# shijun18/H-DenseFormer

Hardware: AMD Instinct MI355X
Metric: train samples/sec on 4x128^3 volumes (higher is better)
Workload: dtype bf16

## Files before the change

h-denseformer_amd/csrc/api_ops.hip:

```cpp
#include <atomic>
#include <algorithm>
#include <cstdarg>
#include <cstring>

#include "../../include/hdf.h"
#include "conv_igemm.h"
#include "loss.h"
#include "optim.h"
#include "transformer.h"
#include "unet_ops.h"

static thread_local char g_err[1024] = "";
static std::atomic<int> g_cu_budget{256};
static int device_cus() {
  static std::atomic<int> cache[16];
  int dev = 0;
  if (hipGetDevice(&dev) != hipSuccess || dev < 0 || dev >= 16) return 256;
  int v = cache[dev].load(std::memory_order_relaxed);
  if (v > 0) return v;
  int n = 0;
  if (hipDeviceGetAttribute(&n, hipDeviceAttributeMultiprocessorCount, dev) != hipSuccess || n <= 0) return 256;
  if (n >= 8) n &= ~7;
  cache[dev].store(n, std::memory_order_relaxed);
  return n;
// ... 386 lines not shown
                          const float* mean, const float* rstd, float* partials, int N, int C, int Do, int Ho, int Wo,
                          hdf_stream stream) {
  HDF_CHECK_ARG(dout && idx && din && y && scale && shift && mean && rstd && partials, "maxpool_bwd_in: null argument");
  return hdf_launch_maxpool_bwd_in(dtype, dout, dout_pitch, idx, din, din_pitch, y, y_pitch, scale, shift, mean, rstd,
                                   partials, N, C, Do, Ho, Wo, (hipStream_t)stream);
}
int hdf_op_upsample_fwd(int dtype, const void* y, int64_t y_pitch, const float* scale, const float* shift, void* out,
                        int64_t out_pitch, int N, int C, int Di, int Hi, int Wi, hdf_stream stream) {
  return hdf_launch_upsample_fwd(dtype, y, y_pitch, scale, shift, out, out_pitch, N, C, Di, Hi, Wi,
                                 (hipStream_t)stream);
}
int hdf_op_upsample_bwd(int dtype, const void* dout, int64_t dout_pitch, void* din, int64_t din_pitch, int N, int C,
                        int Di, int Hi, int Wi, hdf_stream stream) {
  return hdf_launch_upsample_bwd(dtype, dout, dout_pitch, din, din_pitch, N, C, Di, Hi, Wi, (hipStream_t)stream);
}


namespace {
TfDims op_dims(int M, int B, int N, int DM, int64_t mstride, int training, uint64_t seed) {
  TfDims d;
  d.M = M, d.B = B, d.N = N, d.DM = DM, d.DMF = DM + 128;
  d.mstride = mstride;
  d.training = training ? 1 : 0;
  d.seed = (uint32_t)(seed & 0xffffffffu);
  d.thresh24 = 1u << 23;
  d.keep_scale = 2.0f;
  return d;
}
int op_dims_ok(int M, int B, int N, int DM) {
  HDF_CHECK_ARG(M >= 1 && B >= 1 && N >= 1, "transformer op: M=%d B=%d N=%d", M, B, N);
// ... 106 lines not shown
```

h-denseformer_amd/csrc/exec.hip:

```cpp
#include <algorithm>
#include <cstring>
#include <map>
#include <string>

#include "plan_internal.h"
#include "loss.h"
#include "transformer.h"
#include "unet_ops.h"

namespace {

hipStream_t make_stream(bool highest) {
  hipStream_t s = nullptr;
  int least = 0, greatest = 0;
  if (hipDeviceGetStreamPriorityRange(&least, &greatest) != hipSuccess ||
      hipStreamCreateWithPriority(&s, hipStreamNonBlocking, highest ? greatest : least) != hipSuccess) {
    if (hipStreamCreateWithFlags(&s, hipStreamNonBlocking) != hipSuccess) s = nullptr;
  }
  return s;
}

struct Exec {
  hdf_plan* p;
  char* ws;
// ... 692 lines not shown
  void* outs[4] = {out0, out1, out2, out3};
  Xf none;

  static const bool no_branch = getenv("HDF_NO_BRANCH_OVERLAP") != nullptr;
  Exec eb = e;
  hipStream_t bst = no_branch ? nullptr : e.fork_branch();
  if (bst) eb.st = bst, eb.on_branch = true;
  Rejoin rejoin{e, eb, bst != nullptr};
  const bool fused_at3 = !p->flat;
  const int flat = p->flat ? 1 : 0;
  const bool first_direct = bst && p->enc[0][0].Cin <= 4 &&
                            hdf_conv_first_takes(p->dtype, p->enc[0][0].Cin, p->enc[0][0].Cout, p->dims[0][0], p->dims[0][1],
                                                 p->dims[0][2], p->xin.pitch);
  hipStream_t pst = first_direct ? bst : e.st;
  if (first_direct) {
    HDF_TRY(hdf_launch_nchw_to_ndhwc(p->dtype, x, e.at(p->xin), batch, p->M, 16, p->vox(0), e.st));
    HDF_TRY(conv_forward(e, p->enc[0][0], p->xin, none));
  }
  HDF_TRY(hdf_launch_pack_batch(p->dtype, params, e.ws, p->pack_jobs.data(), (int)p->pack_jobs.size(), pst));
  if (p->tf_fwd_chain)
    HDF_TRY(tf_chain_pack(tf_dims(p, batch), tf_chain_params(p), p->nb, params, e.ws + p->tf_wpack, pst));
  hipEvent_t packed = bst ? e.order(pst, e.st, "the caller's stream behind the weight packs", first_direct) : nullptr;
  if (bst && !packed) return HDF_ERR_HIP;
  if (!first_direct) {
    HDF_TRY(hdf_launch_nchw_to_ndhwc(p->dtype, x, e.at(p->xin), batch, p->M, 16, p->vox(0), e.st));
    HDF_TRY(conv_forward(e, p->enc[0][0], p->xin, none));
  }
  const bool chain_first = first_direct && p->tf_fwd_chain;
  eb.tf_packed = first_direct ? nullptr : packed;
  if (chain_first) {
    HDF_TRY(transformer_forward(eb, x));
    if (!e.order(bst, e.st, "the caller's stream behind the branch stream's transformer (tf_done)")) return HDF_ERR_HIP;
  }
  e.conv_budget = (hdf_cu_budget() * 3 / 4) & ~7;
  HDF_TRY(conv_forward(e, p->enc[0][1], p->enc[0][0].y, xf_of(e, p->enc[0][0])));
  e.conv_budget = 0;
  if (!chain_first) HDF_TRY(transformer_forward(eb, x));
  if (packed) HDF_TRY(e.wait(bst, packed, "the branch stream behind the weight packs"));
  HDF_TRY(conv_forward(eb, p->deep, p->attnall, none));
  HDF_TRY(hdf_launch_upsample_fwd(p->dtype, eb.at(p->deep.y), p->deep.y.pitch, eb.f(p->deep.st.scale),
// ... 74 lines not shown
}

static int backward3d(hdf_plan* p, const float* x, const float* params, void* workspace, int64_t workspace_bytes,
                      const void* dout0, const void* dout1, const void* dout2, const void* dout3, float* grads,
                      int batch, int stages, hdf_stream stream, hipEvent_t* bev = nullptr) {
  HDF_CHECK_ARG(p->batch == batch, "backward: batch %d differs from the forward's %d", batch, p->batch);
  HDF_TRY(chain_flag_check(p));
  auto record = [&](int k, hipStream_t s) -> int {
    if (bev && hipEventRecord(bev[k], s) != hipSuccess) {
      hdf_set_error("backward: could not record the event of gradient bucket %d", k);
      return HDF_ERR_HIP;
    }
    return HDF_OK;
  };
  enum { BK_DEC = 0, BK_CHAIN = 1, BK_TF = 2, BK_ENC = 3, BK_ENC0 = 4 };
  auto record_joined = [&](int k, Exec& ex) -> int {
    if (!bev) return HDF_OK;
    if (ex.async && p->side) {
      if (!ex.order(ex.st, p->side, "the side stream behind the issuing stream (gradient bucket event)")) return HDF_ERR_HIP;
      return record(k, p->side);
    }
    return record(k, ex.st);
  };
  HDF_CHECK_ARG((size_t)workspace_bytes >= p->ws_bytes,
                "backward: workspace of %lld bytes holds a forward only (hdf_plan_workspace_bytes = %zu)",
                (long long)workspace_bytes, p->ws_bytes);
  Exec e{p, (char*)workspace, params, grads, batch, (hipStream_t)stream};
  static const bool no_async = getenv("HDF_NO_ASYNC_WGRAD") != nullptr;
  if (!no_async) {
    if (!p->side) p->side = make_stream(false);
// ... 76 lines not shown
      HDF_TRY(hdf_launch_wgrad_first(p->dtype, e.at(p->gA[k]), p->gA[k].pitch, c1.Cout, e.at(p->xin), p->xin.pitch, c1.Cin,
                                     e.B, p->dims[0][0], p->dims[0][1], p->dims[0][2], e.G(c1.w), 0, e.ws + p->wgrad_ws,
                                     p->wgrad_ws_bytes, e.wgrad_stream(), &fi));
      HDF_TRY(e.wgrad_done(p->gA[k]));
      first_fused = true;
    }
    if (!first_fused) {
      if (k > 0)
        HDF_TRY(norm_conv_backward(e, c1, p->gA[k], p->gY2[k], bsr, p->pooled[k - 1], none, &p->dP[k - 1], 0));
      else
        HDF_TRY(norm_conv_backward(e, c1, p->gA[k], p->gY2[k], bsr, p->xin, none, nullptr, 0));
    }
    if (k == 1) HDF_TRY(record_joined(BK_ENC, e));
    if (k == 0 && forked) {
      HDF_TRY(transformer_backward(eb, x));
      if (bev) {
        eb.join();
        HDF_TRY(record(BK_TF, eb.st));
      }
    }
  }

  if (!(stages & 6) || bev) e.join();
  HDF_TRY(record(BK_ENC0, e.st));
  }
  if (forked) {
    HDF_TRY(e.join_branch(eb));
    forked = false;
  } else {
    if (stages & 2) {
      HDF_TRY(upconv_chain_backward(e, batch));
      if (!(stages & 4) || bev) e.join();
      HDF_TRY(record(BK_CHAIN, e.st));
    }
    if (stages & 4) {
      HDF_TRY(transformer_backward(e, x));
      if (bev) {
        e.join();
        HDF_TRY(record(BK_TF, e.st));
      }
    }
  }
  e.join();
  if ((stages & 4) && p->tf_bwd_chain) {
    const unsigned* tmo = reinterpret_cast<const unsigned*>(e.ws + p->tf_sync) + (1 << 17) + p->M * batch * 32;
    hipLaunchKernelGGL(chain_poison_grads_kernel, dim3(1), dim3(256), 0, e.st, tmo, grads,
                       (int)std::min<int64_t>(p->total_floats, 4096));
    HDF_LAUNCH_CHECK();
  }
  return HDF_OK;
}

static int backward_any(hdf_plan* p, const float* x, const float* params, void* workspace, int64_t workspace_bytes,
                        const void* dout0, const void* dout1, const void* dout2, const void* dout3, float* grads,
                        int batch, int stages, hdf_stream stream, hipEvent_t* bev) {
  HDF_CHECK_ARG(p && x && params && workspace && grads, "backward: null argument");
  if (!p->is2d)
    return backward3d(p, x, params, workspace, workspace_bytes, dout0, dout1, dout2, dout3, grads, batch, stages, stream,
                      bev);
  HDF_CHECK_ARG(p->batch == batch && (size_t)workspace_bytes >= p->ws_bytes, "backward: batch / workspace mismatch");
  char* ws = (char*)workspace;
  hipStream_t st = (hipStream_t)stream;
  void* d3[4];
  const void* d2[4] = {dout0, dout1, dout2, dout3};
// ... 141 lines not shown
```

h-denseformer_amd/csrc/plan.hip:

```cpp
#include <cstdarg>
#include <cstring>

#include "plan_internal.h"
#include "transformer.h"

namespace {

void add_param(hdf_plan* p, const std::string& name, std::vector<int64_t> shape) {
  ParamInfo pi;
  pi.name = name;
  pi.shape = shape;
  pi.numel = 1;
  for (auto s : shape) pi.numel *= s;
  pi.offset = p->total_floats;
  p->total_floats += (pi.numel + 15) / 16 * 16;
  p->pidx[name] = (int64_t)p->params.size();
  p->params.push_back(pi);
}

void build_params(hdf_plan* p) {
  const int nf = p->nf, DM = p->DM;
  char buf[256];
  for (int m = 0; m < p->M; m++) {
    int64_t start = p->total_floats;
// ... 151 lines not shown
      Embed2dJob& last = p->ejobs.back();
      if (last.kind == 0 && last.stage == stage && last.off3 + last.n3 == pi.offset && last.off2 + last.n3 == q.offset) {
        last.n3 += n3;
        p->params2d.push_back(q);
        continue;
      }
    }
    p->ejobs.push_back(Embed2dJob{pi.offset, q.offset, n3, inner, (short)rep, (char)kind, stage});
    p->params2d.push_back(q);
  }
  HDF_CHECK_ARG((int)p->ejobs.size() <= HDF_MAX_EMBED_JOBS, "2-D plan: %d embedding jobs (max %d)", (int)p->ejobs.size(),
                HDF_MAX_EMBED_JOBS);
  return HDF_OK;
}

View mkview(hdf_plan* p, Bump& bp, const std::string& name, int lvl, int C, int batch) {
  View v;
  v.C = C;
  v.pitch = C;
  v.lvl = lvl;
  v.off = bp.take((size_t)batch * p->vox(lvl) * C * p->esz);
  if (!name.empty()) p->bufs[name] = v;
  return v;
}

}

View hdf_plan_subview(hdf_plan* p, const View& v, int c0, int C, const std::string& name) {
  View s = v;
  s.off = v.off + (size_t)c0 * p->esz;
// ... 7 lines not shown
  p->batch = B;
  p->bufs.clear();
  Bump bp;
  const int nf = p->nf;
  const int ch[4] = {nf, 2 * nf, 4 * nf, 8 * nf};
  auto conv_bufs = [&](Conv3& c) {
    c.y = mkview(p, bp, "y." + c.name, c.lvl, c.Cout, B);
    size_t s = (size_t)B * c.Cout * sizeof(float);
    c.st.mean = bp.take(s);
    c.st.rstd = bp.take(s);
    c.st.scale = bp.take(s);
    c.st.shift = bp.take(s);
    c.wf = bp.take((size_t)27 * round_up(c.Cout, 32) * c.CinP * p->esz);
    c.wd = bp.take((size_t)27 * round_up(c.CinP, 32) * round_up(c.Cout, 16) * p->esz);
  };
  p->xin = mkview(p, bp, "xin", 0, 16, B);
  const int64_t rows = (int64_t)p->M * B * p->Ntok;
  p->tf_F = bp.take((size_t)p->nb * rows * p->DMF * sizeof(float));
  p->tf_save = bp.take((size_t)p->nb * 4 * rows * 232 * sizeof(float));
  {
    TfDims dd{};
    dd.M = p->M;
    p->tf_wpack = bp.take(tf_chain_wpack_bytes(dd, p->nb));
    dd.B = B, dd.N = p->Ntok;
    p->tf_frag = bp.take(p->dtype == HDF_F32 ? 256 : tf_chain_frag_bytes(dd, p->nb));
  }
  p->tf_sync = bp.take((size_t)3 << 20);
  p->attnall = mkview(p, bp, "attnall", 4, p->M * p->DM, B);
  conv_bufs(p->deep);
  p->attnout = mkview(p, bp, "attnout", 3, 8 * nf, B);
  for (int k = 0; k < 3; k++) conv_bufs(p->up[k]);
// ... 126 lines not shown
  p->D = D, p->H = H, p->W = W;
  p->td = transformer_depth;
  p->nb = transformer_depth / 4;
  p->dtype = dtype;
  p->esz = hdf_esz(dtype);
  for (int l = 0; l < 5; l++) p->dims[l][0] = D >> l, p->dims[l][1] = H >> l, p->dims[l][2] = W >> l;
  p->flat = is2d && flat;
  if (p->flat)
    for (int l = 0; l < 5; l++) p->dims[l][0] = 1;
  p->DM = 4 * n_filters;
  p->DMF = p->DM + 128;
  p->Ntok = (D / 16) * (H / 16) * (W / 16);
  build_params(p);
  build_layers(p);
  p->is2d = is2d;
  if (is2d) {
    int rc = build_params2d(p);
    if (rc != HDF_OK) {
      delete p;
      return rc;
    }
  }
  *out = p;
  return HDF_OK;
}

int hdf_plan_create(int in_channels, int n_cls, int n_filters, int D, int H, int W, int transformer_depth, int dtype,
                    hdf_plan** out) {
  return create_plan(in_channels, n_cls, n_filters, D, H, W, transformer_depth, dtype, false, out);
}
// ... 36 lines not shown
  return (int64_t)p->ws_fwd_bytes;
}

int hdf_plan_buffer_info(hdf_plan* p, int batch, const char* name, int64_t* byte_offset, int64_t* pitch_elems,
                         int* channels, int* d, int* h, int* w) {
  hdf_plan_layout(p, batch);
  auto it = p->bufs.find(name);
  HDF_CHECK_ARG(it != p->bufs.end(), "buffer_info: no buffer named '%s'", name);
  const View& v = it->second;
  *byte_offset = (int64_t)v.off;
  *pitch_elems = v.pitch;
  *channels = v.C;
  *d = p->dims[v.lvl][0];
  *h = p->dims[v.lvl][1];
  *w = p->dims[v.lvl][2];
  return HDF_OK;
}

int hdf_plan_region_info(hdf_plan* p, int batch, const char* name, int64_t* byte_offset, int64_t* bytes) {
  HDF_CHECK_ARG(p && name && byte_offset && bytes, "region_info: null argument");
  hdf_plan_layout(p, batch);
  const int64_t rows = (int64_t)p->M * batch * p->Ntok;
  const std::string n = name;
  if (n == "tf_F") *byte_offset = (int64_t)p->tf_F, *bytes = (int64_t)p->nb * rows * p->DMF * 4;
  else if (n == "tf_save") *byte_offset = (int64_t)p->tf_save, *bytes = (int64_t)p->nb * 4 * rows * 232 * 4;
  else if (n == "tf_sync") *byte_offset = (int64_t)p->tf_sync, *bytes = (int64_t)3 << 20;
  else if (n == "tf_dF") *byte_offset = (int64_t)p->tf_dF, *bytes = rows * p->DMF * 4;
  else if (n == "tf_tape") *byte_offset = (int64_t)p->tf_tape, *bytes = (int64_t)p->nb * 4 * rows * TF_TAPE_W * 4;
  else if (n == "tf_otape") *byte_offset = (int64_t)p->tf_otape, *bytes = (int64_t)p->nb * rows * p->DMF * 4;
  else {
// ... 19 lines not shown
```

h-denseformer_amd/csrc/plan_internal.h:

```cpp
#pragma once
#include <map>
#include <string>
#include <vector>

#include "../../include/hdf.h"
#include "conv_igemm.h"

namespace hdf_internal {

struct ParamInfo {
  std::string name;
  std::vector<int64_t> shape;
  int64_t offset, numel;
};

struct View {
  size_t off = 0;
  int64_t pitch = 0;
  int C = 0;
  int lvl = 0;
};

struct Stats {
  size_t mean = 0, rstd = 0, scale = 0, shift = 0;
// ... 49 lines not shown
  int dims[5][3];
  int DM, DMF, Ntok;
  std::vector<ParamInfo> params;
  std::map<std::string, int64_t> pidx;
  int64_t total_floats = 0;
  int64_t mstride = 0;
  Conv3 deep, up[3], enc[4][2], dec[3][2];
  ConvT3 upc[3];
  Head1 head[4];
  std::vector<PackJob> pack_jobs;
  int batch = -1;
  size_t ws_bytes = 0;
  size_t ws_fwd_bytes = 0;
  std::map<std::string, View> bufs;
  View xin, attnall, attnout, at[3] , cat[3], pooled[3], x4;
  size_t pool_idx[3];
  size_t tf_F, tf_save, tf_scratch, tf_dF, tf_tape = 0, tf_otape = 0;
  size_t tf_sync = 0;
  size_t tf_frag = 0;
  size_t tf_wpack = 0;
  size_t stat_partials, wgrad_ws, inb_partials, inb_k;
  size_t stat_partials2 = 0, inb_partials2 = 0, inb_k2 = 0;
  size_t inb_k3 = 0;
  size_t ksplit_ws = 0, ksplit_ws2 = 0;
  size_t wgrad_ws_bytes = 0;
  View gA[4], gY[4], gY2[4], dCat[3], dUp[3], dSkip[3], dP[3], dUa[4], dUy[4], dX4, dAttnall;
  hipStream_t side = nullptr;
  hipStream_t branch = nullptr;
  std::vector<hipEvent_t> events;
  size_t ev_next = 0;
// ... 42 lines not shown
```

h-denseformer_amd/csrc/unet_ops.h:

```cpp
#pragma once
#include "hdf_common.h"

int hdf_launch_nchw_to_ndhwc(int dtype, const float* x, void* out, int N, int C, int CP, int64_t vox, hipStream_t st);

int hdf_launch_in_finalize(const float* partials, int N, int tiles, int C, int CP, int64_t vox, const float* gamma,
                           const float* beta, float eps, float* mean, float* rstd, float* scale, float* shift,
                           hipStream_t st);

int hdf_launch_norm_relu_add(int dtype, const void* y, int64_t y_pitch, const float* scale, const float* shift,
                             const void* skip, int64_t skip_pitch, void* out, int64_t out_pitch, int N, int C,
                             int64_t vox, hipStream_t st);

int hdf_launch_enc_tail(int dtype, const void* y, int64_t y_pitch, const float* scale, const float* shift,
                        const void* skip, int64_t skip_pitch, void* ds, int64_t ds_pitch, void* pooled,
                        int64_t pooled_pitch, uint8_t* idx, int N, int C, int Do, int Ho, int Wo, hipStream_t st,
                        int flat = 0 );
int hdf_launch_enc_tail_up(int dtype, const void* y, int64_t y_pitch, const float* scale, const float* shift,
                           const void* low, int64_t low_pitch, const float* lscale, const float* lshift, void* ds,
                           int64_t ds_pitch, void* pooled, int64_t pooled_pitch, uint8_t* idx, int N, int C, int Do, int Ho,
                           int Wo, hipStream_t st);
int hdf_launch_maxpool_fwd(int dtype, const void* in, int64_t in_pitch, void* out, int64_t out_pitch, uint8_t* idx,
                           int N, int C, int Do, int Ho, int Wo, hipStream_t st);
int hdf_launch_maxpool_bwd(int dtype, const void* dout, int64_t dout_pitch, const uint8_t* idx, void* din,
                           int64_t din_pitch, int N, int C, int Do, int Ho, int Wo, int accumulate, hipStream_t st);

int hdf_launch_upsample_fwd(int dtype, const void* y, int64_t y_pitch, const float* scale, const float* shift,
                            void* out, int64_t out_pitch, int N, int C, int Di, int Hi, int Wi, hipStream_t st,
                            int flat = 0 );
int hdf_launch_upsample_bwd(int dtype, const void* dout, int64_t dout_pitch, void* din, int64_t din_pitch, int N,
                            int C, int Di, int Hi, int Wi, hipStream_t st, int flat = 0);

int hdf_launch_head_fwd(int dtype, const void* in, int64_t in_pitch, const float* scale, const float* shift,
                        const float* w, const float* b, void* logits, int N, int C, int ncls, int64_t vox,
                        hipStream_t st);
int hdf_head_bwd_blocks(int64_t vox);
int hdf_maxpool_bwd_in_blocks(int64_t pooled_vox, int C);
int hdf_launch_maxpool_bwd_in(int dtype, const void* dout, int64_t dout_pitch, const uint8_t* idx, void* din,
                              int64_t din_pitch, const void* y, int64_t y_pitch, const float* scale, const float* shift,
                              const float* mean, const float* rstd, float* partials, int N, int C, int Do, int Ho, int Wo,
                              hipStream_t st, int flat = 0 );
int hdf_launch_head_bwd(int dtype, const void* dlogits, const void* in, int64_t in_pitch, const float* scale,
                        const float* shift, const float* w, void* dx, int64_t dx_pitch, int accumulate_dx, float* dw,
                        float* db, int N, int C, int ncls, int64_t vox, hipStream_t st, const float* in_mean = nullptr,
                        const float* in_rstd = nullptr, float* inb_partials = nullptr);

// ... 18 lines not shown
```

h-denseformer_amd/csrc/unet_ops.hip:

```cpp
#include "unet_ops.h"

namespace {

constexpr int MAX_BLOCKS = 4096;

template <typename T>
__device__ __forceinline__ void load_chunk(const T* p, float* f) {
  u32x4 v = *reinterpret_cast<const u32x4*>(p);
  ST<T>::unpack(v, f);
}
template <typename T>
__device__ __forceinline__ void store_chunk(T* p, const float* f) {
  *reinterpret_cast<u32x4*>(p) = ST<T>::pack(f);
}

template <typename T>
__global__ void nchw_to_ndhwc_kernel(const float* __restrict__ x, T* __restrict__ out, int N, int C, int CP,
                                     int64_t vox) {
  HDF_LIGHT_PRIO();
  int64_t total = (int64_t)N * vox;
  for (int64_t i = (int64_t)blockIdx.x * blockDim.x + threadIdx.x; i < total; i += (int64_t)gridDim.x * blockDim.x) {
    int64_t n = i / vox, v = i - n * vox;
    for (int c0 = 0; c0 < CP; c0 += ST<T>::EPC) {
      float f[ST<T>::EPC];
#pragma unroll
      for (int e = 0; e < ST<T>::EPC; e++) f[e] = (c0 + e < C) ? x[(n * C + c0 + e) * vox + v] : 0.f;
      store_chunk<T>(out + i * CP + c0, f);
    }
  }
}

constexpr int FIN_LANES = 32, FIN_CG = 8;
__global__ __launch_bounds__(256, 4) void in_finalize_kernel(const float* __restrict__ partials, int tiles, int C, int CP,
                                                           int64_t vox, const float* __restrict__ gamma,
                                                           const float* __restrict__ beta, float eps,
                                                           float* __restrict__ mean, float* __restrict__ rstd,
                                                           float* __restrict__ scale, float* __restrict__ shift) {
  HDF_LIGHT_PRIO();
  __shared__ double red[FIN_LANES][FIN_CG][2];
  const int n = blockIdx.y, cg = blockIdx.x;
  const int cl = threadIdx.x & (FIN_CG - 1), c = cg * FIN_CG + cl, tl = threadIdx.x / FIN_CG;
  double s1 = 0.0, s2 = 0.0;
  if (c < CP) {
// ... 484 lines not shown
    for (int b = 0; b < 4; b++) {
      const float wzy = wz[a] * wy[b];
      const int zy = zo[a] + yo[b];
      float f[4][EPC];
#pragma unroll
      for (int c = 0; c < 4; c++) load_chunk<T>(sbase + (zy + xo[c]), f[c]);
#pragma unroll
      for (int c = 0; c < 4; c++)
#pragma unroll
        for (int e = 0; e < EPC; e++) acc[e] += (wzy * wx[c]) * f[c][e];
    }
  }
  store_chunk<T>(din + (((int64_t)nz * Hi + ih) * Wi + iw) * din_pitch + c0, acc);
}

constexpr int HEAD_MAXCLS = 8;

template <typename T, int MC>
__global__ __launch_bounds__(256) void head_fwd_kernel(const T* __restrict__ in, int64_t in_pitch,
                                                       const float* __restrict__ scale, const float* __restrict__ shift,
                                                       const float* __restrict__ w, const float* __restrict__ b,
                                                       T* __restrict__ logits, int N, int C, int ncls, int64_t vox,
                                                       int per, int vec4) {
  HDF_LIGHT_PRIO();
  constexpr int EPC = ST<T>::EPC;
  extern __shared__ float outs[];
  float* part = outs + MC * per;
  const int n = blockIdx.y;
  const int cols = C / EPC;
  const bool pow2 = (cols & (cols - 1)) == 0 && cols <= 64;
// ... 556 lines not shown
}

static int allow_big_lds(const void* kern, size_t bytes) {
  if (bytes <= 64 * 1024) return HDF_OK;
  hipError_t e = hipFuncSetAttribute(kern, hipFuncAttributeMaxDynamicSharedMemorySize, 160 * 1024);
  if (e != hipSuccess) {
    hdf_set_error("hipFuncSetAttribute(MaxDynamicSharedMemorySize) failed: %s", hipGetErrorString(e));
    return HDF_ERR_HIP;
  }
  return HDF_OK;
}

#define DISPATCH_T HDF_DISPATCH_T

int hdf_launch_nchw_to_ndhwc(int dtype, const float* x, void* out, int N, int C, int CP, int64_t vox, hipStream_t st) {
  HDF_CHECK_ARG(CP % 16 == 0 && CP >= C, "nchw_to_ndhwc: CP=%d", CP);
  DISPATCH_T(dtype, hipLaunchKernelGGL(nchw_to_ndhwc_kernel<T>, dim3(grid_for((int64_t)N * vox)), dim3(256), 0, st, x,
                                       (T*)out, N, C, CP, vox));
  HDF_LAUNCH_CHECK();
  return HDF_OK;
}

__global__ __launch_bounds__(256, 6) void stat_rows_sum_kernel(const float* __restrict__ partials, int rows, int C, int CP,
                                                             float* __restrict__ out) {
  HDF_LIGHT_PRIO();
  __shared__ double red[32][FIN_CG];
  const int cl = threadIdx.x & (FIN_CG - 1), c = blockIdx.x * FIN_CG + cl, rl = threadIdx.x / FIN_CG;
  double s = 0.0;
  if (c < C) {
    const float* p = partials + (int64_t)c * 2;
// ... 199 lines not shown
  HDF_CHECK_ARG(scale && shift, "upsample_fwd: the producer's InstanceNorm scale / shift are required");
  HDF_CHECK_ARG(!flat || Di == 1, "upsample_fwd: the 2-D form takes depth-1 tensors");
  if (flat) {
    DISPATCH_T(dtype, hipLaunchKernelGGL((upsample_fwd_kernel<T, true>),
                                         dim3(grid_for((int64_t)N * Di * Hi * Wi * (C / ST<T>::EPC))), dim3(256), 0, st,
                                         (const T*)y, y_pitch, scale, shift, (T*)out, out_pitch, N, C, Di, Hi, Wi));
  } else {
    DISPATCH_T(dtype, hipLaunchKernelGGL(upsample_fwd_kernel<T>,
                                         dim3(grid_for((int64_t)N * Di * Hi * Wi * (C / ST<T>::EPC))), dim3(256), 0, st,
                                         (const T*)y, y_pitch, scale, shift, (T*)out, out_pitch, N, C, Di, Hi, Wi));
  }
  HDF_LAUNCH_CHECK();
  return HDF_OK;
}

int hdf_launch_upsample_bwd(int dtype, const void* dout, int64_t dout_pitch, void* din, int64_t din_pitch, int N,
                            int C, int Di, int Hi, int Wi, hipStream_t st, int flat) {
  HDF_CHECK_ARG(!flat || Di == 1, "upsample_bwd: the 2-D form takes depth-1 tensors");
  HDF_CHECK_ARG((int64_t)8 * Di * Hi * Wi * dout_pitch < ((int64_t)1 << 31),
                "upsample_bwd: a sample of %dx%dx%d voxels x pitch %lld exceeds 32-bit element offsets", 2 * Di, 2 * Hi,
                2 * Wi, (long long)dout_pitch);
  DISPATCH_T(dtype, {
    const int gx = ceil_div(Wi * (C / ST<T>::EPC), 256);
    const int64_t wgs = (int64_t)gx * Hi * N * Di;
    HDF_CHECK_ARG(wgs < ((int64_t)1 << 31), "upsample_bwd: %lld workgroups", (long long)wgs);
    if (flat)
      hipLaunchKernelGGL((upsample_bwd_kernel<T, true>), dim3((unsigned)wgs), dim3(256), 0, st, (const T*)dout, dout_pitch,
                         (T*)din, din_pitch, N, C, Di, Hi, Wi, gx);
    else
      hipLaunchKernelGGL(upsample_bwd_kernel<T>, dim3((unsigned)wgs), dim3(256), 0, st, (const T*)dout, dout_pitch, (T*)din,
                         din_pitch, N, C, Di, Hi, Wi, gx);
  });
  HDF_LAUNCH_CHECK();
  return HDF_OK;
}

int hdf_launch_head_fwd(int dtype, const void* in, int64_t in_pitch, const float* scale, const float* shift,
                        const float* w, const float* b, void* logits, int N, int C, int ncls, int64_t vox,
                        hipStream_t st) {
  HDF_CHECK_ARG(ncls <= HEAD_MAXCLS, "head: n_cls=%d > %d", ncls, HEAD_MAXCLS);
  HDF_CHECK_ARG(C % 16 == 0 && C <= 1024, "head_fwd: C=%d", C);
  const int per = head_vox(vox, 1024) >= 256 ? head_vox(vox, 1024) : head_vox(vox);
  const unsigned gx = (unsigned)ceil_div64(vox, per);
  const int vec4 = (vox % 4 == 0 && (reinterpret_cast<uintptr_t>(logits) & 15) == 0) ? 1 : 0;
  DISPATCH_T(dtype, {
    auto go = [&](auto kern, int mc) -> int {
      const size_t shm = (size_t)mc * (per + 256) * sizeof(float);
// ... 126 lines not shown
```

h-denseformer_amd/hdf_rt/_lib.py:

```python
import ctypes as C
import os

_HERE = os.path.dirname(os.path.abspath(__file__))
LIB_PATH = os.environ.get("HDF_LIB_PATH") or os.path.join(os.path.dirname(_HERE), "lib", "libhdf_hip.so")

F32, BF16, F16 = 0, 1, 2

_vp, _i, _i64, _f, _u64 = C.c_void_p, C.c_int, C.c_int64, C.c_float, C.c_uint64

_PROTOS = {
    "hdf_version": (C.c_char_p, []),
    "hdf_last_error": (C.c_char_p, []),
    "hdf_set_cu_budget": (_i, [_i]),
    "hdf_plan_create": (_i, [_i] * 8 + [C.POINTER(_vp)]),
    "hdf_plan_create_2d": (_i, [_i] * 7 + [C.POINTER(_vp)]),
    "hdf_plan_create_2d_embedded": (_i, [_i] * 7 + [C.POINTER(_vp)]),
    "hdf_plan_destroy": (None, [_vp]),
    "hdf_plan_num_params": (_i64, [_vp]),
    "hdf_plan_param_floats": (_i64, [_vp]),
    "hdf_plan_param_info": (_i, [_vp, _i64, C.c_char_p, _i, C.POINTER(_i64), C.POINTER(_i64), C.POINTER(_i),
                                 C.POINTER(_i64)]),
    "hdf_plan_workspace_bytes": (_i64, [_vp, _i]),
    "hdf_plan_inference_workspace_bytes": (_i64, [_vp, _i]),
    "hdf_plan_buffer_info": (_i, [_vp, _i, C.c_char_p, C.POINTER(_i64), C.POINTER(_i64), C.POINTER(_i),
                                  C.POINTER(_i), C.POINTER(_i), C.POINTER(_i)]),
    "hdf_plan_region_info": (_i, [_vp, _i, C.c_char_p, C.POINTER(_i64), C.POINTER(_i64)]),
    "hdf_forward": (_i, [_vp, _vp, _vp, _vp, _i64, _vp, _vp, _vp, _vp, _i, _i, _u64, _vp]),
    "hdf_backward": (_i, [_vp, _vp, _vp, _vp, _i64, _vp, _vp, _vp, _vp, _vp, _i, _vp]),
    "hdf_backward_stages": (_i, [_vp, _vp, _vp, _vp, _i64, _vp, _vp, _vp, _vp, _vp, _i, _i, _vp]),
    "hdf_backward_events": (_i, [_vp, _vp, _vp, _vp, _i64, _vp, _vp, _vp, _vp, _vp, _i, _vp, C.POINTER(_vp)]),
    "hdf_plan_grad_bucket": (_i, [_vp, _i, C.POINTER(_i64), C.POINTER(_i64)]),
    "hdf_stream_wait_event": (_i, [_vp, _vp]),
    "hdf_plan_set_probe": (_i, [_vp, _vp, _vp]),
    "hdf_plan_set_chain_timeout_us": (_i, [_vp, _i64]),
    "hdf_plan_chain_state": (_i, [_vp, _i, C.POINTER(_i), C.POINTER(_i)]),
    "hdf_plan_force_persistent": (_i, [_vp, _i]),
    "hdf_op_occupy": (_i, [_i, _i, _i, _i, _vp]),
    "hdf_loss_workspace_bytes": (_i64, [_i]),
    "hdf_loss_forward": (_i, [_i, _vp, _vp, _vp, _vp, _i, _vp, _i, _i, _i, _i, _i, _vp, _vp, _vp]),
    "hdf_loss_backward": (_i, [_i, _vp, _vp, _vp, _vp, _i, _vp, _i, _i, _i, _i, _i, _vp, _vp, _vp, _vp, _vp, _vp,
                               _vp]),
    "hdf_loss_terms_forward": (_i, [_i, _vp, _vp, _vp, _vp, _i, _vp, _i, _i, _i, _i, _i, _f, _f, _vp, _vp, _vp]),
    "hdf_loss_terms_backward": (_i, [_i, _vp, _vp, _vp, _vp, _i, _vp, _i, _i, _i, _i, _i, _f, _f, _vp, _vp, _vp, _vp,
                                     _vp, _vp, _vp]),
    "hdf_loss_weighted_forward": (_i, [_i, _vp, _vp, _vp, _vp, _i, _vp, _i, _i, _i, _i, _i, _f, _f, _vp, _i, _vp, _vp,
                                       _vp]),
    "hdf_loss_weighted_backward": (_i, [_i, _vp, _vp, _vp, _vp, _i, _vp, _i, _i, _i, _i, _i, _f, _f, _vp, _i, _vp, _vp,
                                        _vp, _vp, _vp, _vp, _vp]),
    "hdf_loss_focal_forward": (_i, [_i, _vp, _vp, _vp, _vp, _i, _vp, _i, _i, _i, _i, _i, _f, _f, _f, _i, _f, _vp, _i,
                                    _vp, _vp, _vp]),
    "hdf_loss_focal_backward": (_i, [_i, _vp, _vp, _vp, _vp, _i, _vp, _i, _i, _i, _i, _i, _f, _f, _f, _i, _f, _vp, _i,
# ... 29 lines not shown
    "hdf_op_in_bwd_wgrad": (_i, [_i, _vp, _i64, _vp, _i64, _vp, _vp, _vp, _vp, _vp, _vp, _i64, _vp, _vp, _vp, _i64, _i,
                                 _vp, _vp, _i, _i, _i, _i, _i, _i, _vp, _vp, _vp, _i64, _vp]),
    "hdf_op_conv3d_wgrad": (_i, [_i, _i, _vp, _i64, _i, _vp, _i64, _i, _i, _i, _i, _i, _vp, _vp, _i, _vp, _vp, _i,
                                 _vp, _i, _i, _i, _vp, _i64, _vp]),
    "hdf_op_in_finalize": (_i, [_vp, _i, _i, _i, _i, _i64, _vp, _vp, _f, _vp, _vp, _vp, _vp, _vp]),
    "hdf_op_norm_relu_add": (_i, [_i, _vp, _i64, _vp, _vp, _vp, _i64, _vp, _i64, _i, _i, _i64, _vp]),
    "hdf_op_maxpool_fwd": (_i, [_i, _vp, _i64, _vp, _i64, _vp, _i, _i, _i, _i, _i, _vp]),
    "hdf_op_maxpool_bwd_in_rows": (_i, [_i, _i, _i, _i]),
    "hdf_op_maxpool_bwd_in": (_i, [_i, _vp, _i64, _vp, _vp, _i64, _vp, _i64, _vp, _vp, _vp, _vp, _vp, _i, _i, _i, _i, _i, _vp]),
    "hdf_op_enc_tail": (_i, [_i, _vp, _i64, _vp, _vp, _vp, _i64, _vp, _i64, _vp, _i64, _vp, _i, _i, _i, _i, _i, _vp]),
    "hdf_op_enc_tail_up": (_i, [_i, _vp, _i64, _vp, _vp, _vp, _i64, _vp, _vp, _vp, _i64, _vp, _i64, _vp, _i, _i, _i, _i, _i,
                                _vp]),
    "hdf_op_maxpool_bwd": (_i, [_i, _vp, _i64, _vp, _vp, _i64, _i, _i, _i, _i, _i, _i, _vp]),
    "hdf_op_upsample_fwd": (_i, [_i, _vp, _i64, _vp, _vp, _vp, _i64, _i, _i, _i, _i, _i, _vp]),
    "hdf_op_upsample_bwd": (_i, [_i, _vp, _i64, _vp, _i64, _i, _i, _i, _i, _i, _vp]),
    "hdf_op_attention_fwd": (_i, [_vp, _i, _i, _vp, _vp, _vp]),
    "hdf_op_attention_bwd": (_i, [_vp, _vp, _vp, _vp, _vp, _i, _i, _vp]),
    "hdf_op_attention_amp_bwd": (_i, [_i, _vp, _vp, _vp, _vp, _vp, _i, _i, _vp]),
    "hdf_op_patch_embed_fwd": (_i, [_vp, _i, _i, _i, _i, _i, _i, _vp, _vp, _vp, _i64, _vp, _i, _u64, _vp]),
    "hdf_op_patch_embed_bwd": (_i, [_vp, _i, _i, _i, _i, _i, _i, _vp, _i64, _vp, _vp, _vp, _vp, _i, _u64, _vp]),
    "hdf_op_dense_layer_fwd": (_i, [_i, _i, _i, _i, _i, _i, _vp, _i64, _vp, _vp, _i, _u64, _vp]),
    "hdf_op_dense_layer_bwd": (_i, [_i, _i, _i, _i, _i, _i, _vp, _vp, _i64, _vp, _vp, _vp, _vp, _i, _u64, _vp]),
    "hdf_op_block_out_fwd": (_i, [_i, _i, _i, _i, _i, _vp, _i64, _vp, _vp, _vp, _i, _i, _u64, _vp]),
    "hdf_op_block_out_bwd": (_i, [_i, _i, _i, _i, _i, _vp, _vp, _i64, _vp, _vp, _vp, _i, _vp, _i, _u64, _vp]),
    "hdf_op_head_fwd": (_i, [_i, _vp, _i64, _vp, _vp, _vp, _vp, _vp, _i, _i, _i, _i64, _vp]),
    "hdf_op_head_bwd": (_i, [_i, _vp, _vp, _i64, _vp, _vp, _vp, _vp, _i64, _i, _vp, _vp, _i, _i, _i, _i64, _vp]),
}

EXPORTS = tuple(_PROTOS.keys())

# ... 41 lines not shown
```

include/hdf.h:

```cpp
#ifndef HDF_H
#define HDF_H
#include <stddef.h>
#include <stdint.h>

#ifdef __cplusplus
extern "C" {
#endif

typedef struct hdf_plan hdf_plan;
typedef void* hdf_stream;

const char* hdf_version(void);
const char* hdf_last_error(void);
int hdf_set_cu_budget(int cus);

int hdf_plan_create(int in_channels, int n_cls, int n_filters, int D, int H, int W, int transformer_depth, int dtype,
                    hdf_plan** out);
int hdf_plan_create_2d(int in_channels, int n_cls, int n_filters, int H, int W, int transformer_depth, int dtype,
                       hdf_plan** out);
int hdf_plan_create_2d_embedded(int in_channels, int n_cls, int n_filters, int H, int W, int transformer_depth, int dtype,
                                hdf_plan** out);
void hdf_plan_destroy(hdf_plan* p);
int64_t hdf_plan_num_params(const hdf_plan* p);
int64_t hdf_plan_param_floats(const hdf_plan* p);
// ... 13 lines not shown
                 hdf_stream stream);

int hdf_backward_stages(hdf_plan* p, const float* x, const float* params, void* workspace, int64_t workspace_bytes,
                        const void* dout0, const void* dout1, const void* dout2, const void* dout3, float* grads,
                        int batch, int stages, hdf_stream stream);

#define HDF_NUM_GRAD_BUCKETS 5
int hdf_plan_grad_bucket(const hdf_plan* p, int k, int64_t* lo, int64_t* hi);
int hdf_backward_events(hdf_plan* p, const float* x, const float* params, void* workspace, int64_t workspace_bytes,
                        const void* dout0, const void* dout1, const void* dout2, const void* dout3, float* grads,
                        int batch, hdf_stream stream, void** bucket_events );
#define HDF_ERR_CHAIN_TIMEOUT 4
int hdf_plan_set_chain_timeout_us(hdf_plan* p, int64_t usec);
int hdf_plan_chain_state(hdf_plan* p, int batch, int* persistent, int* gave_up_workgroup);
int hdf_plan_force_persistent(hdf_plan* p, int on);
int hdf_op_occupy(int workgroups, int lds_bytes, int vgprs, int usec, hdf_stream stream);

int hdf_plan_set_probe(hdf_plan* p, void* ev_start, void* ev_stop);
int hdf_stream_wait_event(hdf_stream stream, void* event);

int64_t hdf_loss_workspace_bytes(int batch);
int hdf_loss_forward(int dtype, const void* out0, const void* out1, const void* out2, const void* out3, int nscale,
                     const float* target_onehot, int batch, int n_cls, int D, int H, int W, void* workspace,
                     float* loss_out, hdf_stream stream);
int hdf_loss_backward(int dtype, const void* out0, const void* out1, const void* out2, const void* out3, int nscale,
                      const float* target_onehot, int batch, int n_cls, int D, int H, int W, const void* workspace,
                      const float* grad_out, void* dout0, void* dout1, void* dout2, void* dout3, hdf_stream stream);
int hdf_loss_terms_forward(int dtype, const void* out0, const void* out1, const void* out2, const void* out3, int nscale,
                           const float* target_onehot, int batch, int n_cls, int D, int H, int W, float ce_weight,
                           float dice_weight, void* workspace, float* loss_out, hdf_stream stream);
// ... 116 lines not shown
int hdf_op_enc_tail_up(int dtype, const void* y, int64_t y_pitch, const float* scale, const float* shift, const void* low,
                       int64_t low_pitch, const float* lscale, const float* lshift, void* ds, int64_t ds_pitch,
                       void* pooled, int64_t pooled_pitch, uint8_t* idx, int N, int C, int Do, int Ho, int Wo,
                       hdf_stream stream);
int hdf_op_maxpool_bwd(int dtype, const void* dout, int64_t dout_pitch, const uint8_t* idx, void* din,
                       int64_t din_pitch, int N, int C, int Do, int Ho, int Wo, int accumulate, hdf_stream stream);
int hdf_op_maxpool_bwd_in_rows(int C, int Do, int Ho, int Wo);
int hdf_op_maxpool_bwd_in(int dtype, const void* dout, int64_t dout_pitch, const uint8_t* idx, void* din,
                          int64_t din_pitch, const void* y, int64_t y_pitch, const float* scale, const float* shift,
                          const float* mean, const float* rstd, float* partials, int N, int C, int Do, int Ho, int Wo,
                          hdf_stream stream);
int hdf_op_upsample_fwd(int dtype, const void* y, int64_t y_pitch, const float* scale, const float* shift, void* out,
                        int64_t out_pitch, int N, int C, int Di, int Hi, int Wi, hdf_stream stream);
int hdf_op_upsample_bwd(int dtype, const void* dout, int64_t dout_pitch, void* din, int64_t din_pitch, int N, int C,
                        int Di, int Hi, int Wi, hdf_stream stream);



int hdf_op_attention_fwd(const float* qkv, int nseq, int N, float* ob, float* lse, hdf_stream stream);
int hdf_op_attention_bwd(const float* qkv, const float* ob, const float* lse, const float* d_ob, float* dqkv, int nseq,
                         int N, hdf_stream stream);
int hdf_op_attention_amp_bwd(int dtype, const float* qkv, const float* ob, const float* lse, const float* d_ob,
                             float* dqkv, int nseq, int N, hdf_stream stream);
int hdf_op_patch_embed_fwd(const float* x, int M, int B, int D, int H, int W, int DM, const float* weight,
                           const float* bias, const float* pos, int64_t mstride, float* F, int training, uint64_t seed,
                           hdf_stream stream);
int hdf_op_patch_embed_bwd(const float* x, int M, int B, int D, int H, int W, int DM, const float* dF, int64_t mstride,
                           float* dweight, float* dbias, float* dpos, float* scratch, int training, uint64_t seed,
                           hdf_stream stream);
int hdf_op_dense_layer_fwd(int M, int B, int N, int DM, int block, int layer, const float* const* params13,
// ... 22 lines not shown
```

Measured before the change: 187.2.

## Use 4-channel input rows, add blocked upsample backward, move chain poison launch

Pads the network input to 4 channels instead of 16 when the first conv and its weight-gradient kernels accept that pitch, and adds a dedicated NCHW-to-NDHWC kernel for 4-channel rows. This cuts input transform traffic and first-layer memory. It also adds a register-blocked upsample backward kernel with selectable forms, but the default route returns form 0, so training still uses the old kernel. The poison-grads launch now runs right after each transformer backward on that stream, not after the final join.

```diff
diff --git a/h-denseformer_amd/csrc/api_ops.hip b/h-denseformer_amd/csrc/api_ops.hip
--- a/h-denseformer_amd/csrc/api_ops.hip
+++ b/h-denseformer_amd/csrc/api_ops.hip
@@ -424,6 +424,11 @@
                         int Di, int Hi, int Wi, hdf_stream stream) {
   return hdf_launch_upsample_bwd(dtype, dout, dout_pitch, din, din_pitch, N, C, Di, Hi, Wi, (hipStream_t)stream);
 }
+int hdf_op_upsample_bwd_form(int dtype, const void* dout, int64_t dout_pitch, void* din, int64_t din_pitch, int N, int C,
+                             int Di, int Hi, int Wi, int flat, int form, hdf_stream stream) {
+  HDF_CHECK_ARG(hdf_upsample_bwd_form_ok(form, flat), "upsample_bwd_form: form %d (flat %d)", form, flat);
+  return hdf_launch_upsample_bwd(dtype, dout, dout_pitch, din, din_pitch, N, C, Di, Hi, Wi, (hipStream_t)stream, flat, form);
+}
 
 
 namespace {
diff --git a/h-denseformer_amd/csrc/exec.hip b/h-denseformer_amd/csrc/exec.hip
--- a/h-denseformer_amd/csrc/exec.hip
+++ b/h-denseformer_amd/csrc/exec.hip
@@ -730,7 +730,7 @@
                                                  p->dims[0][2], p->xin.pitch);
   hipStream_t pst = first_direct ? bst : e.st;
   if (first_direct) {
-    HDF_TRY(hdf_launch_nchw_to_ndhwc(p->dtype, x, e.at(p->xin), batch, p->M, 16, p->vox(0), e.st));
+    HDF_TRY(hdf_launch_nchw_to_ndhwc(p->dtype, x, e.at(p->xin), batch, p->M, (int)p->xin.pitch, p->vox(0), e.st));
     HDF_TRY(conv_forward(e, p->enc[0][0], p->xin, none));
   }
   HDF_TRY(hdf_launch_pack_batch(p->dtype, params, e.ws, p->pack_jobs.data(), (int)p->pack_jobs.size(), pst));
@@ -739,7 +739,7 @@
   hipEvent_t packed = bst ? e.order(pst, e.st, "the caller's stream behind the weight packs", first_direct) : nullptr;
   if (bst && !packed) return HDF_ERR_HIP;
   if (!first_direct) {
-    HDF_TRY(hdf_launch_nchw_to_ndhwc(p->dtype, x, e.at(p->xin), batch, p->M, 16, p->vox(0), e.st));
+    HDF_TRY(hdf_launch_nchw_to_ndhwc(p->dtype, x, e.at(p->xin), batch, p->M, (int)p->xin.pitch, p->vox(0), e.st));
     HDF_TRY(conv_forward(e, p->enc[0][0], p->xin, none));
   }
   const bool chain_first = first_direct && p->tf_fwd_chain;
@@ -844,6 +844,14 @@
     return HDF_OK;
   };
   enum { BK_DEC = 0, BK_CHAIN = 1, BK_TF = 2, BK_ENC = 3, BK_ENC0 = 4 };
+  auto poison = [&](Exec& ex) -> int {
+    if (!p->tf_bwd_chain) return HDF_OK;
+    const unsigned* tmo = reinterpret_cast<const unsigned*>(ex.ws + p->tf_sync) + (1 << 17) + p->M * batch * 32;
+    hipLaunchKernelGGL(chain_poison_grads_kernel, dim3(1), dim3(256), 0, ex.st, tmo, grads,
+                       (int)std::min<int64_t>(p->total_floats, 4096));
+    HDF_LAUNCH_CHECK();
+    return HDF_OK;
+  };
   auto record_joined = [&](int k, Exec& ex) -> int {
     if (!bev) return HDF_OK;
     if (ex.async && p->side) {
@@ -950,6 +958,7 @@
     if (k == 1) HDF_TRY(record_joined(BK_ENC, e));
     if (k == 0 && forked) {
       HDF_TRY(transformer_backward(eb, x));
+      HDF_TRY(poison(eb));
       if (bev) {
         eb.join();
         HDF_TRY(record(BK_TF, eb.st));
@@ -971,6 +980,7 @@
     }
     if (stages & 4) {
       HDF_TRY(transformer_backward(e, x));
+      HDF_TRY(poison(e));
       if (bev) {
         e.join();
         HDF_TRY(record(BK_TF, e.st));
@@ -978,12 +988,6 @@
     }
   }
   e.join();
-  if ((stages & 4) && p->tf_bwd_chain) {
-    const unsigned* tmo = reinterpret_cast<const unsigned*>(e.ws + p->tf_sync) + (1 << 17) + p->M * batch * 32;
-    hipLaunchKernelGGL(chain_poison_grads_kernel, dim3(1), dim3(256), 0, e.st, tmo, grads,
-                       (int)std::min<int64_t>(p->total_floats, 4096));
-    HDF_LAUNCH_CHECK();
-  }
   return HDF_OK;
 }
 
diff --git a/h-denseformer_amd/csrc/plan.hip b/h-denseformer_amd/csrc/plan.hip
--- a/h-denseformer_amd/csrc/plan.hip
+++ b/h-denseformer_amd/csrc/plan.hip
@@ -189,6 +189,14 @@
   return HDF_OK;
 }
 
+int input_row_channels(const hdf_plan* p) {
+  const Conv3& c = p->enc[0][0];
+  const int* d = p->dims[0];
+  const bool narrow = !p->is2d && c.Cin <= 4 && hdf_conv_first_takes(p->dtype, c.Cin, c.Cout, d[0], d[1], d[2], 4) &&
+                      hdf_wgrad_first_takes(p->dtype, c.Cin, c.Cout, d[0], d[1], d[2], 4, c.Cout);
+  return narrow ? 4 : 16;
+}
+
 View mkview(hdf_plan* p, Bump& bp, const std::string& name, int lvl, int C, int batch) {
   View v;
   v.C = C;
@@ -226,7 +234,7 @@
     c.wf = bp.take((size_t)27 * round_up(c.Cout, 32) * c.CinP * p->esz);
     c.wd = bp.take((size_t)27 * round_up(c.CinP, 32) * round_up(c.Cout, 16) * p->esz);
   };
-  p->xin = mkview(p, bp, "xin", 0, 16, B);
+  p->xin = mkview(p, bp, "xin", 0, p->xin_cp, B);
   const int64_t rows = (int64_t)p->M * B * p->Ntok;
   p->tf_F = bp.take((size_t)p->nb * rows * p->DMF * sizeof(float));
   p->tf_save = bp.take((size_t)p->nb * 4 * rows * 232 * sizeof(float));
@@ -383,6 +391,7 @@
   build_params(p);
   build_layers(p);
   p->is2d = is2d;
+  p->xin_cp = input_row_channels(p);
   if (is2d) {
     int rc = build_params2d(p);
     if (rc != HDF_OK) {
@@ -449,6 +458,13 @@
   *d = p->dims[v.lvl][0];
   *h = p->dims[v.lvl][1];
   *w = p->dims[v.lvl][2];
+  return HDF_OK;
+}
+
+int hdf_plan_force_wide_input(hdf_plan* p, int on) {
+  HDF_CHECK_ARG(p != nullptr, "force_wide_input: null plan");
+  const int cp = on ? 16 : input_row_channels(p);
+  if (cp != p->xin_cp) p->xin_cp = cp, p->batch = -1;
   return HDF_OK;
 }
 
diff --git a/h-denseformer_amd/csrc/plan_internal.h b/h-denseformer_amd/csrc/plan_internal.h
--- a/h-denseformer_amd/csrc/plan_internal.h
+++ b/h-denseformer_amd/csrc/plan_internal.h
@@ -87,6 +87,7 @@
   size_t ws_fwd_bytes = 0;
   std::map<std::string, View> bufs;
   View xin, attnall, attnout, at[3] , cat[3], pooled[3], x4;
+  int xin_cp = 16;
   size_t pool_idx[3];
   size_t tf_F, tf_save, tf_scratch, tf_dF, tf_tape = 0, tf_otape = 0;
   size_t tf_sync = 0;
diff --git a/h-denseformer_amd/csrc/unet_ops.h b/h-denseformer_amd/csrc/unet_ops.h
--- a/h-denseformer_amd/csrc/unet_ops.h
+++ b/h-denseformer_amd/csrc/unet_ops.h
@@ -28,7 +28,9 @@
                             void* out, int64_t out_pitch, int N, int C, int Di, int Hi, int Wi, hipStream_t st,
                             int flat = 0 );
 int hdf_launch_upsample_bwd(int dtype, const void* dout, int64_t dout_pitch, void* din, int64_t din_pitch, int N,
-                            int C, int Di, int Hi, int Wi, hipStream_t st, int flat = 0);
+                            int C, int Di, int Hi, int Wi, hipStream_t st, int flat = 0,
+                            int form = -1 );
+bool hdf_upsample_bwd_form_ok(int form, int flat);
 
 int hdf_launch_head_fwd(int dtype, const void* in, int64_t in_pitch, const float* scale, const float* shift,
                         const float* w, const float* b, void* logits, int N, int C, int ncls, int64_t vox,
diff --git a/h-denseformer_amd/csrc/unet_ops.hip b/h-denseformer_amd/csrc/unet_ops.hip
--- a/h-denseformer_amd/csrc/unet_ops.hip
+++ b/h-denseformer_amd/csrc/unet_ops.hip
@@ -27,6 +27,28 @@
       for (int e = 0; e < ST<T>::EPC; e++) f[e] = (c0 + e < C) ? x[(n * C + c0 + e) * vox + v] : 0.f;
       store_chunk<T>(out + i * CP + c0, f);
     }
+  }
+}
+
+template <typename T>
+__global__ __launch_bounds__(256) void nchw_to_ndhwc4_kernel(const float* __restrict__ x, T* __restrict__ out, int C,
+                                                             int64_t vox) {
+  HDF_LIGHT_PRIO();
+  const int n = blockIdx.y;
+  const float* const xs = x + (int64_t)n * C * vox;
+  T* const os = out + (int64_t)n * vox * 4;
+  const int64_t v0 = (int64_t)blockIdx.x * 1024 + threadIdx.x;
+  float f[4][4];
+#pragma unroll
+  for (int j = 0; j < 4; j++) {
+    const int64_t v = v0 + 256 * j;
+#pragma unroll
+    for (int c = 0; c < 4; c++) f[j][c] = (c < C && v < vox) ? xs[c * vox + v] : 0.f;
+  }
+#pragma unroll
+  for (int j = 0; j < 4; j++) {
+    const int64_t v = v0 + 256 * j;
+    if (v < vox) ST<T>::st4(os + v * 4, f[j][0], f[j][1], f[j][2], f[j][3]);
   }
 }
 
@@ -541,6 +563,98 @@
   store_chunk<T>(din + (((int64_t)nz * Hi + ih) * Wi + iw) * din_pitch + c0, acc);
 }
 
+__device__ __forceinline__ float up_bwd_w(int i, int n, int q) {
+  return q == 0 ? (i >= 1 ? 0.25f : 0.f) : q == 1 ? (i == 0 ? 1.0f : 0.75f) : q == 2 ? (i == n - 1 ? 1.0f : 0.75f)
+                                                                                   : (i <= n - 2 ? 0.25f : 0.f);
+}
+
+template <typename T, bool FLAT, int BZ, int BY, int BX>
+__global__ __launch_bounds__(256) void upsample_bwd_blk_kernel(const T* __restrict__ dout, int64_t dout_pitch,
+                                                               T* __restrict__ din, int64_t din_pitch, int N, int C, int Di,
+                                                               int Hi, int Wi, int gx) {
+  static_assert(!FLAT || BZ == 1, "the 2-D form has one plane");
+  HDF_LIGHT_PRIO();
+  constexpr int EPC = ST<T>::EPC;
+  constexpr int UZ = FLAT ? 1 : 2 * BZ + 2, UY = 2 * BY + 2, UX = 2 * BX + 2, ROWS = UZ * UY;
+  static_assert(ROWS % 2 == 0, "the row loop takes two rows per trip");
+  const int cols = C / EPC;
+  const int Do = (FLAT ? 1 : 2) * Di, Ho = 2 * Hi, Wo = 2 * Wi;
+  const int DB = (Di + BZ - 1) / BZ, HB = (Hi + BY - 1) / BY, WB = (Wi + BX - 1) / BX;
+  const int vb = xcd_slab_id(blockIdx.x, gridDim.x);
+  const int xt = vb % gx, r = vb / gx;
+  const int ih0 = (r % HB) * BY, nzb = r / HB;
+  const int id0 = (nzb % DB) * BZ, n = nzb / DB;
+  const int t = xt * 256 + threadIdx.x;
+  if (t >= WB * cols) return;
+  const int bw = t / cols, c0 = (t - bw * cols) * EPC, iw0 = bw * BX;
+  float wx[BX][4];
+  {
+    int o[4];
+#pragma unroll
+    for (int k = 0; k < BX; k++) up_bwd_taps(iw0 + k, Wi, o, wx[k]);
+  }
+  const T* const sbase = dout + (int64_t)n * Do * Ho * Wo * dout_pitch + c0;
+  const int pit = (int)dout_pitch;
+  int xo[UX];
+#pragma unroll
+  for (int u = 0; u < UX; u++) xo[u] = min(max(2 * iw0 - 1 + u, 0), Wo - 1) * pit;
+  float acc[BZ][BY][BX][EPC];
+#pragma unroll
+  for (int i = 0; i < BZ * BY * BX * EPC; i++) (&acc[0][0][0][0])[i] = 0.f;
+  auto load_row = [&](int row, u32x4* dst) __attribute__((always_inline)) {
+    const int uz = row / UY, uy = row - uz * UY;
+    const int zy = (FLAT ? 0 : min(max(2 * id0 - 1 + uz, 0), Do - 1) * Ho * Wo * pit) +
+                   min(max(2 * ih0 - 1 + uy, 0), Ho - 1) * Wo * pit;
+#pragma unroll
+    for (int ux = 0; ux < UX; ux++) dst[ux] = *reinterpret_cast<const u32x4*>(sbase + (zy + xo[ux]));
+  };
+  auto fma_row = [&](int row, const u32x4* src) __attribute__((always_inline)) {
+    const int uz = row / UY, uy = row - uz * UY;
+#pragma unroll
+    for (int bz = 0; bz < BZ; bz++) {
+#pragma unroll
+      for (int by = 0; by < BY; by++) {
+        const int a = uz - 2 * bz, b = uy - 2 * by;
+        if ((unsigned)a < (FLAT ? 1u : 4u) && (unsigned)b < 4u) {
+          const float wzy = (FLAT ? 1.f : up_bwd_w(id0 + bz, Di, a)) * up_bwd_w(ih0 + by, Hi, b);
+#pragma unroll
+          for (int ux = 0; ux < UX; ux++) {
+            float f[EPC];
+            ST<T>::unpack(src[ux], f);
+#pragma unroll
+            for (int bx = 0; bx < BX; bx++) {
+              const int c = ux - 2 * bx;
+              if (c < 0 || c > 3) continue;
+              const float w = wzy * wx[bx][c];
+#pragma unroll
+              for (int e = 0; e < EPC; e++) acc[bz][by][bx][e] = __builtin_fmaf(w, f[e], acc[bz][by][bx][e]);
+            }
+          }
+        }
+      }
+    }
+  };
+  u32x4 r0[UX], r1[UX];
+  load_row(0, r0);
+#pragma unroll 1
+  for (int row = 0; row < ROWS; row += 2) {
+    load_row(row + 1, r1);
+    fma_row(row, r0);
+    load_row(min(row + 2, ROWS - 1), r0);
+    fma_row(row + 1, r1);
+  }
+  T* const obase = din + ((((int64_t)n * Di + id0) * Hi + ih0) * Wi + iw0) * din_pitch + c0;
+  const int op = (int)din_pitch;
+#pragma unroll
+  for (int bz = 0; bz < BZ; bz++)
+#pragma unroll
+    for (int by = 0; by < BY; by++)
+#pragma unroll
+      for (int bx = 0; bx < BX; bx++)
+        if (id0 + bz < Di && ih0 + by < Hi && iw0 + bx < Wi)
+          store_chunk<T>(obase + (int64_t)((bz * Hi + by) * Wi + bx) * op, acc[bz][by][bx]);
+}
+
 constexpr int HEAD_MAXCLS = 8;
 
 template <typename T, int MC>
@@ -1127,6 +1241,18 @@
 #define DISPATCH_T HDF_DISPATCH_T
 
 int hdf_launch_nchw_to_ndhwc(int dtype, const float* x, void* out, int N, int C, int CP, int64_t vox, hipStream_t st) {
+  if (CP == 4 && dtype != HDF_F32) {
+    HDF_CHECK_ARG(C >= 1 && C <= 4 && N >= 1 && N <= 65535 && vox >= 1 && ceil_div64(vox, 1024) < ((int64_t)1 << 31),
+                  "nchw_to_ndhwc: 4-channel rows take C = 1..4 (C=%d, N=%d)", C, N);
+    HDF_CHECK_ARG((reinterpret_cast<uintptr_t>(out) & 7) == 0, "nchw_to_ndhwc: output must be 8-byte aligned");
+    const dim3 grid((unsigned)ceil_div64(vox, 1024), N);
+    if (dtype == HDF_BF16)
+      hipLaunchKernelGGL(nchw_to_ndhwc4_kernel<bf16_t>, grid, dim3(256), 0, st, x, (bf16_t*)out, C, vox);
+    else
+      hipLaunchKernelGGL(nchw_to_ndhwc4_kernel<f16_t>, grid, dim3(256), 0, st, x, (f16_t*)out, C, vox);
+    HDF_LAUNCH_CHECK();
+    return HDF_OK;
+  }
   HDF_CHECK_ARG(CP % 16 == 0 && CP >= C, "nchw_to_ndhwc: CP=%d", CP);
   DISPATCH_T(dtype, hipLaunchKernelGGL(nchw_to_ndhwc_kernel<T>, dim3(grid_for((int64_t)N * vox)), dim3(256), 0, st, x,
                                        (T*)out, N, C, CP, vox));
@@ -1356,23 +1482,41 @@
   return HDF_OK;
 }
 
+bool hdf_upsample_bwd_form_ok(int form, int flat) {
+  return form == 0 || form == 122 || (!flat && (form == 221 || form == 222));
+}
+
+static int upsample_bwd_route(int , int , int , int , int , int ) { return 0; }
+
+#define UPB_ARGS (const T*)dout, dout_pitch, (T*)din, din_pitch, N, C, Di, Hi, Wi, gx
 int hdf_launch_upsample_bwd(int dtype, const void* dout, int64_t dout_pitch, void* din, int64_t din_pitch, int N,
-                            int C, int Di, int Hi, int Wi, hipStream_t st, int flat) {
+                            int C, int Di, int Hi, int Wi, hipStream_t st, int flat, int form) {
   HDF_CHECK_ARG(!flat || Di == 1, "upsample_bwd: the 2-D form takes depth-1 tensors");
   HDF_CHECK_ARG((int64_t)8 * Di * Hi * Wi * dout_pitch < ((int64_t)1 << 31),
                 "upsample_bwd: a sample of %dx%dx%d voxels x pitch %lld exceeds 32-bit element offsets", 2 * Di, 2 * Hi,
                 2 * Wi, (long long)dout_pitch);
+  HDF_CHECK_ARG(form == -1 || hdf_upsample_bwd_form_ok(form, flat), "upsample_bwd: form %d (flat %d)", form, flat);
   DISPATCH_T(dtype, {
-    const int gx = ceil_div(Wi * (C / ST<T>::EPC), 256);
-    const int64_t wgs = (int64_t)gx * Hi * N * Di;
-    HDF_CHECK_ARG(wgs < ((int64_t)1 << 31), "upsample_bwd: %lld workgroups", (long long)wgs);
-    if (flat)
-      hipLaunchKernelGGL((upsample_bwd_kernel<T, true>), dim3((unsigned)wgs), dim3(256), 0, st, (const T*)dout, dout_pitch,
-                         (T*)din, din_pitch, N, C, Di, Hi, Wi, gx);
+    if (form < 0) form = upsample_bwd_route(N, C, Di, Hi, Wi, flat);
+    const int bz = form / 100, by = form / 10 % 10, bx = form % 10;
+    const int gx = ceil_div(ceil_div(Wi, std::max(bx, 1)) * (C / ST<T>::EPC), 256);
+    const int64_t wgs = (int64_t)gx * ceil_div(Hi, std::max(by, 1)) * N * ceil_div(Di, std::max(bz, 1));
+    HDF_CHECK_ARG(wgs >= 1 && wgs < ((int64_t)1 << 31), "upsample_bwd: %lld workgroups", (long long)wgs);
+    const dim3 grid((unsigned)wgs);
+    if (form == 0 && flat)
+      hipLaunchKernelGGL((upsample_bwd_kernel<T, true>), grid, dim3(256), 0, st, UPB_ARGS);
+    else if (form == 0)
+      hipLaunchKernelGGL(upsample_bwd_kernel<T>, grid, dim3(256), 0, st, UPB_ARGS);
+    else if (flat)
+      hipLaunchKernelGGL((upsample_bwd_blk_kernel<T, true, 1, 2, 2>), grid, dim3(256), 0, st, UPB_ARGS);
+    else if (form == 122)
+      hipLaunchKernelGGL((upsample_bwd_blk_kernel<T, false, 1, 2, 2>), grid, dim3(256), 0, st, UPB_ARGS);
+    else if (form == 221)
+      hipLaunchKernelGGL((upsample_bwd_blk_kernel<T, false, 2, 2, 1>), grid, dim3(256), 0, st, UPB_ARGS);
     else
-      hipLaunchKernelGGL(upsample_bwd_kernel<T>, dim3((unsigned)wgs), dim3(256), 0, st, (const T*)dout, dout_pitch, (T*)din,
-                         din_pitch, N, C, Di, Hi, Wi, gx);
+      hipLaunchKernelGGL((upsample_bwd_blk_kernel<T, false, 2, 2, 2>), grid, dim3(256), 0, st, UPB_ARGS);
   });
+#undef UPB_ARGS
   HDF_LAUNCH_CHECK();
   return HDF_OK;
 }
diff --git a/h-denseformer_amd/hdf_rt/_lib.py b/h-denseformer_amd/hdf_rt/_lib.py
--- a/h-denseformer_amd/hdf_rt/_lib.py
+++ b/h-denseformer_amd/hdf_rt/_lib.py
@@ -35,6 +35,7 @@
     "hdf_plan_set_chain_timeout_us": (_i, [_vp, _i64]),
     "hdf_plan_chain_state": (_i, [_vp, _i, C.POINTER(_i), C.POINTER(_i)]),
     "hdf_plan_force_persistent": (_i, [_vp, _i]),
+    "hdf_plan_force_wide_input": (_i, [_vp, _i]),
     "hdf_op_occupy": (_i, [_i, _i, _i, _i, _vp]),
     "hdf_loss_workspace_bytes": (_i64, [_i]),
     "hdf_loss_forward": (_i, [_i, _vp, _vp, _vp, _vp, _i, _vp, _i, _i, _i, _i, _i, _vp, _vp, _vp]),
@@ -94,6 +95,7 @@
     "hdf_op_maxpool_bwd": (_i, [_i, _vp, _i64, _vp, _vp, _i64, _i, _i, _i, _i, _i, _i, _vp]),
     "hdf_op_upsample_fwd": (_i, [_i, _vp, _i64, _vp, _vp, _vp, _i64, _i, _i, _i, _i, _i, _vp]),
     "hdf_op_upsample_bwd": (_i, [_i, _vp, _i64, _vp, _i64, _i, _i, _i, _i, _i, _vp]),
+    "hdf_op_upsample_bwd_form": (_i, [_i, _vp, _i64, _vp, _i64, _i, _i, _i, _i, _i, _i, _i, _vp]),
     "hdf_op_attention_fwd": (_i, [_vp, _i, _i, _vp, _vp, _vp]),
     "hdf_op_attention_bwd": (_i, [_vp, _vp, _vp, _vp, _vp, _i, _i, _vp]),
     "hdf_op_attention_amp_bwd": (_i, [_i, _vp, _vp, _vp, _vp, _vp, _i, _i, _vp]),
diff --git a/include/hdf.h b/include/hdf.h
--- a/include/hdf.h
+++ b/include/hdf.h
@@ -51,6 +51,7 @@
 int hdf_plan_set_chain_timeout_us(hdf_plan* p, int64_t usec);
 int hdf_plan_chain_state(hdf_plan* p, int batch, int* persistent, int* gave_up_workgroup);
 int hdf_plan_force_persistent(hdf_plan* p, int on);
+int hdf_plan_force_wide_input(hdf_plan* p, int on);
 int hdf_op_occupy(int workgroups, int lds_bytes, int vgprs, int usec, hdf_stream stream);
 
 int hdf_plan_set_probe(hdf_plan* p, void* ev_start, void* ev_stop);
@@ -197,6 +198,8 @@
                         int64_t out_pitch, int N, int C, int Di, int Hi, int Wi, hdf_stream stream);
 int hdf_op_upsample_bwd(int dtype, const void* dout, int64_t dout_pitch, void* din, int64_t din_pitch, int N, int C,
                         int Di, int Hi, int Wi, hdf_stream stream);
+int hdf_op_upsample_bwd_form(int dtype, const void* dout, int64_t dout_pitch, void* din, int64_t din_pitch, int N, int C,
+                             int Di, int Hi, int Wi, int flat, int form, hdf_stream stream);
 
 
 
```

Measured after the change: 188.8, median of 6. No clear change (+0.8%).
